# scale-lab/MTLoRA

Hardware: AMD Instinct MI355X
Metric: images/sec (train step) Swin-T/448 r=64 4-task (higher is better)
Workload: dtype bf16; 1 GPU; BASELINE configs[1]: Swin-T 448, 4 tasks (semseg,normals,sal,human_parts), r_shared=64 r_task=4 scale4; train step (fwd+loss+bwd+clip+AdamW), dropout .05, drop_path .2; per_gpu_batch=32, global_batch=32, img_size=448, parallelism=dp1, trainable_params=8344634, allreduce_bytes=0

## Files before the change

include/mtlora_hip.h:

```cpp
#ifndef MTLORA_HIP_H
#define MTLORA_HIP_H

#include <stdint.h>

#ifdef __cplusplus
extern "C" {
#endif

#define MTLORA_ABI_VERSION 12
#define MTLORA_MAX_TASKS 8

typedef enum mtlora_dtype {
    MTLORA_F32 = 0,
    MTLORA_BF16 = 1,
    MTLORA_F16 = 2,
    MTLORA_U8 = 3
} mtlora_dtype;

typedef enum mtlora_status {
    MTLORA_OK = 0,
    MTLORA_ERR_DTYPE = -1,
    MTLORA_ERR_SHAPE = -2,
    MTLORA_ERR_ALIGN = -3,
    MTLORA_ERR_NULL = -4,
// ... 23 lines not shown
    int32_t T;
    int32_t r_s;
    int32_t r_t[MTLORA_MAX_TASKS];
    float scale_s;
    float scale_t[MTLORA_MAX_TASKS];
    int32_t has_x_tasks;
    float dropout_p;
    uint64_t seed;
    const uint64_t* seed_offset;
    int32_t bwd_phase;
    int32_t sel_stream;
    int32_t sel_dense;
    int32_t sel_tn;
    int32_t sel_projk;
    int32_t max_cu;
    const void* packed;
    int32_t hid;
    int32_t hid_pad_;
    const void* hid_ptr;
} mtlora_linear_desc;

#define MTLORA_HID_FWD_BASE 1
#define MTLORA_HID_P_GIVEN 2
#define MTLORA_HID_Q_GIVEN 4

int64_t mtlora_linear_ctx_bytes(const mtlora_linear_desc* d);

int64_t mtlora_linear_packed_bytes(const mtlora_linear_desc* d);
int mtlora_linear_pack(const mtlora_linear_desc* d, const float* A_s, const float* B_s, const float* const* A_t,
                       const float* const* B_t, void* packed, int64_t packed_bytes, void* stream);
int64_t mtlora_linear_pack_entry_bytes(void);
int mtlora_linear_pack_entry(const mtlora_linear_desc* d, const float* A_s, const float* B_s, const float* const* A_t,
                             const float* const* B_t, void* packed, int64_t packed_bytes, void* entry_host);
int mtlora_linear_pack_table(const void* table_dev, int n_entries, int dtype, void* stream);
int64_t mtlora_linear_bwd_scratch_bytes(const mtlora_linear_desc* d);

int mtlora_linear_fwd(const mtlora_linear_desc* d, const void* x, const void* const* x_t, const void* W,
                      const float* bias, const float* A_s, const float* B_s, const float* const* A_t,
                      const float* const* B_t, void* y_s, void* const* y_t, void* ctx, int64_t ctx_bytes,
                      void* stream);

int mtlora_linear_bwd(const mtlora_linear_desc* d, const void* x, const void* const* x_t, const void* Wt,
                      const void* dy_s, const void* const* dy_t, const void* ctx, int64_t ctx_bytes, void* dx,
                      void* const* dx_t, float* dA_s, float* dB_s, float* const* dA_t, float* const* dB_t,
                      void* scratch, int64_t scratch_bytes, void* stream);

int mtlora_linear_fwd_gelu(const mtlora_linear_desc* d, const void* x, const void* const* x_t, const void* W,
                           const float* bias, const float* A_s, const float* B_s, const float* const* A_t,
                           const float* const* B_t, void* y_s, void* const* y_t, void* a_s, void* const* a_t, void* ctx,
                           int64_t ctx_bytes, void* stream);

int mtlora_linear_bwd_gelu(const mtlora_linear_desc* d, const void* x, const void* const* x_t, const void* Wt,
                           const void* dy_s, const void* const* dy_t, const void* ctx, int64_t ctx_bytes, void* dx,
                           void* const* dx_t, float* dA_s, float* dB_s, float* const* dA_t, float* const* dB_t,
                           void* scratch, int64_t scratch_bytes, const void* h_s, const void* const* h_t, void* stream);

int mtlora_mlp_hid_supported(const mtlora_linear_desc* d1, const mtlora_linear_desc* d2);
int64_t mtlora_mlp_hid_fwd_scratch_bytes(const mtlora_linear_desc* d1, const mtlora_linear_desc* d2);
int64_t mtlora_mlp_hid_bwd_scratch_bytes(const mtlora_linear_desc* d1, const mtlora_linear_desc* d2);
int mtlora_mlp_hid_proj(const mtlora_linear_desc* d1, const mtlora_linear_desc* d2, const void* h_base, const void* ctx1,
                        void* ctx2, void* scratch, int64_t scratch_bytes, void* stream);
int mtlora_mlp_hid_bwd(const mtlora_linear_desc* d1, const mtlora_linear_desc* d2, const void* h_base, const void* dh_s,
                       const void* ctx1, const void* ctx2, const void* scratch2, void* scratch1, void* g, float* const* dB1_t,
                       float* const* dA2_t, void* part, int64_t part_bytes, void* stream);

int64_t mtlora_gemm_tn_scratch_bytes(int64_t M, int Na, int Nb);
int mtlora_gemm_tn(const void* a, const void* b, float* out, int64_t M, int Na, int Nb, int64_t lda, int64_t ldb,
                   int dtype, void* scratch, int64_t scratch_bytes, void* stream);

typedef struct mtlora_attn_desc {
    int64_t B;
    int32_t H, W;
    int32_t window_size;
    int32_t shift;
    int32_t num_heads;
    int32_t head_dim;
    int32_t image_layout;
    int32_t dtype;
    float scale;
    float mask_value;
} mtlora_attn_desc;

int64_t mtlora_window_attn_bwd_scratch_bytes(const mtlora_attn_desc* d);

int mtlora_window_attn_fwd(const mtlora_attn_desc* d, const void* qkv, const float* bias, const float* mask,
                           const int32_t* mask_ids, void* out, void* stream);
int mtlora_window_attn_bwd(const mtlora_attn_desc* d, const void* qkv, const float* bias, const float* mask,
                           const int32_t* mask_ids, const void* dout, void* dqkv, float* dbias, void* scratch,
                           int64_t scratch_bytes, void* stream);

typedef struct mtlora_attn_dropout {
    float p;
    uint64_t seed;
    const uint64_t* seed_offset;
} mtlora_attn_dropout;
int mtlora_window_attn_drop_fwd(const mtlora_attn_desc* d, const mtlora_attn_dropout* drop, const void* qkv, const float* bias,
                                const float* mask, const int32_t* mask_ids, void* out, void* stream);
int mtlora_window_attn_drop_bwd(const mtlora_attn_desc* d, const mtlora_attn_dropout* drop, const void* qkv, const float* bias,
                                const float* mask, const int32_t* mask_ids, const void* dout, void* dqkv, float* dbias, void* scratch,
                                int64_t scratch_bytes, void* stream);

int mtlora_layernorm_fwd(const void* x, const float* gamma, const float* beta, void* y, float* mean, float* rstd,
                         int64_t M, int64_t C, float eps, int x_dtype, int y_dtype, int merge_h, int merge_w, void* stream);
int64_t mtlora_layernorm_bwd_scratch_bytes(int64_t M, int64_t C, int x_dtype);
int mtlora_layernorm_bwd(const void* dy, const void* x, const float* gamma, const float* mean, const float* rstd,
                         void* dx, float* dgamma, float* dbeta, int64_t M, int64_t C, int x_dtype, int dy_dtype,
                         void* scratch, int64_t scratch_bytes, const void* dx_addend, int merge_h, int merge_w, void* stream);

int mtlora_residual_layernorm_fwd(const void* shortcut, const void* branch, const float* scale, int64_t B, const float* gamma,
                                  const float* beta, void* x_new, void* y, float* mean, float* rstd, int64_t M, int64_t C,
                                  float eps, int x_dtype, int y_dtype, void* stream);
int mtlora_residual_layernorm_bwd(const void* dy, const void* x_new, const float* gamma, const float* mean, const float* rstd,
                                  void* d_shortcut, void* d_branch, float* dgamma, float* dbeta, const float* scale,
                                  int64_t B, int64_t M, int64_t C, int x_dtype, int dy_dtype, void* scratch,
                                  int64_t scratch_bytes, const void* dx_addend, void* stream);

int64_t mtlora_layernorm_multi_bwd_scratch_bytes(int n, int64_t M, int64_t C, int x_dtype);
int mtlora_layernorm_multi_fwd(int n, const void* const* x, const float* gamma, const float* beta, void* const* y,
                               float* const* mean, float* const* rstd, int64_t M, int64_t C, float eps, int x_dtype, int y_dtype,
                               int merge_h, int merge_w, void* stream);
int mtlora_layernorm_multi_bwd(int n, const void* const* dy, const void* const* x, const float* gamma, const float* const* mean,
                               const float* const* rstd, void* const* dx, float* dgamma, float* dbeta, int64_t M, int64_t C,
                               int x_dtype, int dy_dtype, void* scratch, int64_t scratch_bytes, const void* const* dx_addend,
                               int merge_h, int merge_w, void* stream);

int mtlora_residual_layernorm_streams_fwd(int n, const void* const* res, const void* const* branch, const float* scale,
                                          int64_t B, const float* gamma, const float* beta, void* const* x_new, void* const* y,
                                          float* const* mean, float* const* rstd, int64_t M, int64_t C, float eps, int x_dtype,
                                          int y_dtype, int merge_h, int merge_w, void* stream);
int mtlora_residual_layernorm_streams_bwd(int n, const void* const* dy, const void* const* x_new, const float* gamma,
                                          const float* const* mean, const float* const* rstd, void* const* d_res,
                                          void* const* d_branch, float* dgamma, float* dbeta, const float* scale, int64_t B,
                                          int64_t M, int64_t C, int x_dtype, int dy_dtype, void* scratch, int64_t scratch_bytes,
                                          const void* const* dx_addend, int merge_h, int merge_w, void* stream);

int mtlora_residual_layernorm_multi_fwd(int n, const void* shortcut, const void* const* branch, const float* scale, int64_t B,
                                        const float* gamma, const float* beta, void* const* x_new, void* const* y,
                                        float* const* mean, float* const* rstd, int64_t M, int64_t C, float eps, int x_dtype,
                                        int y_dtype, void* stream);
int mtlora_residual_layernorm_multi_bwd(int n, const void* const* dy, const void* const* x_new, const float* gamma,
                                        const float* const* mean, const float* const* rstd, const void* const* dx_addend,
                                        void* d_shortcut, void* const* d_branch, float* dgamma, float* dbeta, const float* scale,
                                        int64_t B, int64_t M, int64_t C, int x_dtype, int dy_dtype, void* scratch,
                                        int64_t scratch_bytes, void* stream);

int64_t mtlora_bn_scratch_bytes(int64_t R, int64_t C, int dtype);
int mtlora_bn_relu_fwd(const void* x, const float* gamma, const float* beta, float* running_mean, float* running_var,
                       float momentum, float eps, int relu, void* y, float* save_mean, float* save_rstd,
                       float* save_scale, float* save_shift, int64_t R, int64_t C, int dtype, void* scratch,
                       int64_t scratch_bytes, void* stream);
int mtlora_bn_relu_bwd(const void* dy, const void* x, const float* save_mean, const float* save_rstd,
                       const float* save_scale, const float* save_shift, int relu, void* dx, float* dgamma, float* dbeta,
                       int64_t R, int64_t C, int dtype, void* scratch, int64_t scratch_bytes, void* stream);

int mtlora_residual_droppath_fwd(int n, const void* const* res, const void* const* y, void* const* out,
                                 const float* scale, int64_t M, int64_t C, int64_t B, int res_dtype, int y_dtype,
                                 void* stream);
int mtlora_residual_droppath_bwd(int n, const void* const* g, void* const* dy, void* dres, const float* scale,
                                 int64_t M, int64_t C, int64_t B, int res_dtype, int y_dtype, void* stream);

int64_t mtlora_upsample_loss_partials(int64_t B, int h, int w, int scale);
int mtlora_upsample_loss(int kind, const void* low, const float* label, const float* stat, void* dlow, float* partials,
                         int64_t B, int h, int w, int C, int scale, int dtype, float ignore_index, void* stream);

int mtlora_upsample_metrics_sizes(int kind, int64_t B, int h, int w, int C, int scale, int64_t* n_int64,
                                  int64_t* n_float_partials);
// ... 188 lines not shown
```

mtlora_amd/_lib.py:

```python
from __future__ import annotations

import ctypes
import os
from ctypes import POINTER, Structure, c_char_p, c_double, c_float, c_int, c_int32, c_int64, c_uint64, c_void_p

import torch

MAX_TASKS = 8
ABI_VERSION = 12
F32, BF16, F16, U8 = 0, 1, 2, 3
_DT = {torch.float32: F32, torch.bfloat16: BF16, torch.float16: F16}

_HERE = os.path.dirname(os.path.abspath(__file__))
LIB_PATH = os.path.join(_HERE, "csrc", "libmtlora_hip.so")


class LinearDesc(Structure):
    _fields_ = [("M", c_int64), ("K", c_int64), ("N", c_int64), ("dtype", c_int32), ("mode", c_int32),
                ("T", c_int32), ("r_s", c_int32), ("r_t", c_int32 * MAX_TASKS), ("scale_s", c_float),
                ("scale_t", c_float * MAX_TASKS), ("has_x_tasks", c_int32), ("dropout_p", c_float),
                ("seed", c_uint64), ("seed_offset", c_void_p), ("bwd_phase", c_int32),
                ("sel_stream", c_int32), ("sel_dense", c_int32), ("sel_tn", c_int32), ("sel_projk", c_int32),
                ("max_cu", c_int32), ("packed", c_void_p),
                ("hid", c_int32), ("hid_pad_", c_int32), ("hid_ptr", c_void_p)]
# ... 40 lines not shown
    _fields_ = [("kind", c_int64), ("warmup_t", c_int64), ("warmup_prefix", c_int64), ("t_initial", c_int64), ("decay_t", c_int64),
                ("n_milestones", c_int64), ("milestones", c_int64 * 16), ("warmup_lr_init", c_double), ("lr_min", c_double),
                ("lr_min_rate", c_double), ("decay_rate", c_double), ("gamma", c_double), ("base_lr", c_double * 16)]


class IngestJob(Structure):
    _fields_ = [("src", c_void_p), ("dst", c_void_p), ("kind", c_int32), ("src_dtype", c_int32), ("C", c_int32),
                ("reserved", c_int32)]


class AugmentJob(Structure):
    _fields_ = [("src", c_void_p), ("dst", c_void_p), ("kind", c_int32), ("flags", c_int32)]


class MeterSource(Structure):
    _fields_ = [("src", c_void_p), ("dtype", c_int32), ("reserved", c_int32), ("weight", c_double), ("period", c_int64)]


METER_MAX_SLOTS, METER_F32, METER_F64 = 64, 0, 1
INGEST_MAX_JOBS = 8
AUGMENT_IMAGE_CUBIC_U8, AUGMENT_CLASS_NEAREST_U8, AUGMENT_NORMALS_CUBIC_F32, AUGMENT_DEPTH_NEAREST_F32 = 0, 1, 2, 3
AUGMENT_GEOM_BITS, AUGMENT_FLAG_NO_RENORM = 24, 1
INGEST_IMAGE, INGEST_CLASS, INGEST_CLASS_ALLZERO_IGNORE, INGEST_NORMALS, INGEST_DEPTH = 0, 1, 2, 3, 4

ADAMW_CHUNK, ADAMW_MAX_GROUPS, ADAMW_CTRL_WORDS = 4096, 16, 64
ADAMW_GROUPS_DEV_BYTES = 1152
ADAMW_CTRL_MICRO, ADAMW_CTRL_UPDATED = 5, 6
ADAMW_MAX_ACCUM_STEPS = 1 << 24
LR_MAX_MILESTONES = 16
LR_COSINE, LR_STEP, LR_LINEAR, LR_MULTISTEP = 1, 2, 3, 4
ADAMW_SCHED_COUNT_OFFSET, ADAMW_SCHED_LR_OFFSET, ADAMW_SCHED_DEV_BYTES = 344, 352, 480
SNAPSHOT_CHUNK = 32768

PROF_KINDS = 24


class ProfSummary(Structure):
    _fields_ = [("count", c_int64 * PROF_KINDS), ("ms", ctypes.c_double * PROF_KINDS),
                ("alg_bytes", ctypes.c_double * PROF_KINDS), ("s8d_bytes", ctypes.c_double * PROF_KINDS),
                ("flops", ctypes.c_double * PROF_KINDS)]


PtrArr = c_void_p * MAX_TASKS
PtrArr9 = c_void_p * (MAX_TASKS + 1)

_SIGS = {
    "mtlora_version": (c_int, []),
    "mtlora_error_string": (c_char_p, [c_int]),
    "mtlora_roll_and_window_partition_forward": (c_int, [c_void_p, c_void_p, c_int64, c_int64, c_int64, c_int64, c_int, c_int, c_int, c_void_p]),
    "mtlora_roll_and_window_partition_backward": (c_int, [c_void_p, c_void_p, c_int64, c_int64, c_int64, c_int64, c_int, c_int, c_int, c_void_p]),
    "mtlora_window_merge_and_roll_forward": (c_int, [c_void_p, c_void_p, c_int64, c_int64, c_int64, c_int64, c_int, c_int, c_int, c_void_p]),
    "mtlora_window_merge_and_roll_backward": (c_int, [c_void_p, c_void_p, c_int64, c_int64, c_int64, c_int64, c_int, c_int, c_int, c_void_p]),
    "mtlora_linear_ctx_bytes": (c_int64, [POINTER(LinearDesc)]),
    "mtlora_linear_bwd_scratch_bytes": (c_int64, [POINTER(LinearDesc)]),
    "mtlora_linear_packed_bytes": (c_int64, [POINTER(LinearDesc)]),
    "mtlora_linear_pack": (c_int, [POINTER(LinearDesc), c_void_p, c_void_p, POINTER(c_void_p), POINTER(c_void_p), c_void_p, c_int64,
                                   c_void_p]),
    "mtlora_linear_pack_entry_bytes": (c_int64, []),
    "mtlora_linear_pack_entry": (c_int, [POINTER(LinearDesc), c_void_p, c_void_p, POINTER(c_void_p), POINTER(c_void_p), c_void_p, c_int64,
                                         c_void_p]),
    "mtlora_linear_pack_table": (c_int, [c_void_p, c_int, c_int, c_void_p]),
    "mtlora_linear_fwd": (c_int, [POINTER(LinearDesc), c_void_p, POINTER(c_void_p), c_void_p, c_void_p, c_void_p, c_void_p,
                                  POINTER(c_void_p), POINTER(c_void_p), c_void_p, POINTER(c_void_p), c_void_p, c_int64,
                                  c_void_p]),
    "mtlora_linear_bwd": (c_int, [POINTER(LinearDesc), c_void_p, POINTER(c_void_p), c_void_p, c_void_p, POINTER(c_void_p),
                                  c_void_p, c_int64, c_void_p, POINTER(c_void_p), c_void_p, c_void_p, POINTER(c_void_p),
                                  POINTER(c_void_p), c_void_p, c_int64, c_void_p]),
    "mtlora_gemm_tn_scratch_bytes": (c_int64, [c_int64, c_int, c_int]),
    "mtlora_gemm_tn": (c_int, [c_void_p, c_void_p, c_void_p, c_int64, c_int, c_int, c_int64, c_int64, c_int, c_void_p, c_int64,
                               c_void_p]),
    "mtlora_linear_fwd_gelu": (c_int, [POINTER(LinearDesc), c_void_p, POINTER(c_void_p), c_void_p, c_void_p, c_void_p, c_void_p,
                                       POINTER(c_void_p), POINTER(c_void_p), c_void_p, POINTER(c_void_p), c_void_p,
                                       POINTER(c_void_p), c_void_p, c_int64, c_void_p]),
    "mtlora_linear_bwd_gelu": (c_int, [POINTER(LinearDesc), c_void_p, POINTER(c_void_p), c_void_p, c_void_p, POINTER(c_void_p),
                                       c_void_p, c_int64, c_void_p, POINTER(c_void_p), c_void_p, c_void_p, POINTER(c_void_p),
                                       POINTER(c_void_p), c_void_p, c_int64, c_void_p, POINTER(c_void_p), c_void_p]),
    "mtlora_mlp_hid_supported": (c_int, [POINTER(LinearDesc), POINTER(LinearDesc)]),
    "mtlora_mlp_hid_bwd_scratch_bytes": (c_int64, [POINTER(LinearDesc), POINTER(LinearDesc)]),
    "mtlora_mlp_hid_fwd_scratch_bytes": (c_int64, [POINTER(LinearDesc), POINTER(LinearDesc)]),
    "mtlora_mlp_hid_proj": (c_int, [POINTER(LinearDesc), POINTER(LinearDesc), c_void_p, c_void_p, c_void_p, c_void_p, c_int64, c_void_p]),
    "mtlora_mlp_hid_bwd": (c_int, [POINTER(LinearDesc), POINTER(LinearDesc), c_void_p, c_void_p, c_void_p, c_void_p, c_void_p, c_void_p,
                                   c_void_p, POINTER(c_void_p), POINTER(c_void_p), c_void_p, c_int64, c_void_p]),
    "mtlora_window_attn_bwd_scratch_bytes": (c_int64, [POINTER(AttnDesc)]),
    "mtlora_window_attn_fwd": (c_int, [POINTER(AttnDesc), c_void_p, c_void_p, c_void_p, c_void_p, c_void_p, c_void_p]),
    "mtlora_window_attn_bwd": (c_int, [POINTER(AttnDesc), c_void_p, c_void_p, c_void_p, c_void_p, c_void_p, c_void_p,
                                       c_void_p, c_void_p, c_int64, c_void_p]),
    "mtlora_window_attn_drop_fwd": (c_int, [POINTER(AttnDesc), POINTER(AttnDropout), c_void_p, c_void_p, c_void_p, c_void_p, c_void_p,
                                            c_void_p]),
    "mtlora_window_attn_drop_bwd": (c_int, [POINTER(AttnDesc), POINTER(AttnDropout), c_void_p, c_void_p, c_void_p, c_void_p, c_void_p,
                                            c_void_p, c_void_p, c_void_p, c_int64, c_void_p]),
    "mtlora_layernorm_fwd": (c_int, [c_void_p, c_void_p, c_void_p, c_void_p, c_void_p, c_void_p, c_int64, c_int64, c_float,
                                     c_int, c_int, c_int, c_int, c_void_p]),
    "mtlora_layernorm_bwd_scratch_bytes": (c_int64, [c_int64, c_int64, c_int]),
    "mtlora_residual_layernorm_fwd": (c_int, [c_void_p, c_void_p, c_void_p, c_int64, c_void_p, c_void_p, c_void_p, c_void_p,
                                              c_void_p, c_void_p, c_int64, c_int64, c_float, c_int, c_int, c_void_p]),
    "mtlora_layernorm_multi_bwd_scratch_bytes": (c_int64, [c_int, c_int64, c_int64, c_int]),
    "mtlora_layernorm_multi_fwd": (c_int, [c_int, POINTER(c_void_p), c_void_p, c_void_p, POINTER(c_void_p), POINTER(c_void_p),
                                           POINTER(c_void_p), c_int64, c_int64, c_float, c_int, c_int, c_int, c_int, c_void_p]),
    "mtlora_layernorm_multi_bwd": (c_int, [c_int, POINTER(c_void_p), POINTER(c_void_p), c_void_p, POINTER(c_void_p),
                                           POINTER(c_void_p), POINTER(c_void_p), c_void_p, c_void_p, c_int64, c_int64, c_int,
                                           c_int, c_void_p, c_int64, POINTER(c_void_p), c_int, c_int, c_void_p]),
    "mtlora_residual_layernorm_streams_fwd": (c_int, [c_int, POINTER(c_void_p), POINTER(c_void_p), c_void_p, c_int64, c_void_p,
                                                      c_void_p, POINTER(c_void_p), POINTER(c_void_p), POINTER(c_void_p),
                                                      POINTER(c_void_p), c_int64, c_int64, c_float, c_int, c_int, c_int, c_int,
                                                      c_void_p]),
    "mtlora_residual_layernorm_streams_bwd": (c_int, [c_int, POINTER(c_void_p), POINTER(c_void_p), c_void_p, POINTER(c_void_p),
                                                      POINTER(c_void_p), POINTER(c_void_p), POINTER(c_void_p), c_void_p, c_void_p,
                                                      c_void_p, c_int64, c_int64, c_int64, c_int, c_int, c_void_p, c_int64,
                                                      POINTER(c_void_p), c_int, c_int, c_void_p]),
    "mtlora_residual_layernorm_multi_fwd": (c_int, [c_int, c_void_p, POINTER(c_void_p), c_void_p, c_int64, c_void_p, c_void_p,
                                                    POINTER(c_void_p), POINTER(c_void_p), POINTER(c_void_p), POINTER(c_void_p),
                                                    c_int64, c_int64, c_float, c_int, c_int, c_void_p]),
    "mtlora_residual_layernorm_multi_bwd": (c_int, [c_int, POINTER(c_void_p), POINTER(c_void_p), c_void_p, POINTER(c_void_p),
                                                    POINTER(c_void_p), POINTER(c_void_p), c_void_p, POINTER(c_void_p), c_void_p,
                                                    c_void_p, c_void_p, c_int64, c_int64, c_int64, c_int, c_int, c_void_p, c_int64,
                                                    c_void_p]),
    "mtlora_residual_layernorm_bwd": (c_int, [c_void_p, c_void_p, c_void_p, c_void_p, c_void_p, c_void_p, c_void_p, c_void_p,
                                              c_void_p, c_void_p, c_int64, c_int64, c_int64, c_int, c_int, c_void_p, c_int64,
                                              c_void_p, c_void_p]),
    "mtlora_layernorm_bwd": (c_int, [c_void_p, c_void_p, c_void_p, c_void_p, c_void_p, c_void_p, c_void_p, c_void_p,
                                     c_int64, c_int64, c_int, c_int, c_void_p, c_int64, c_void_p, c_int, c_int, c_void_p]),
    "mtlora_bn_scratch_bytes": (c_int64, [c_int64, c_int64, c_int]),
    "mtlora_bn_relu_fwd": (c_int, [c_void_p, c_void_p, c_void_p, c_void_p, c_void_p, c_float, c_float, c_int, c_void_p,
                                   c_void_p, c_void_p, c_void_p, c_void_p, c_int64, c_int64, c_int, c_void_p, c_int64,
                                   c_void_p]),
    "mtlora_bn_relu_bwd": (c_int, [c_void_p, c_void_p, c_void_p, c_void_p, c_void_p, c_void_p, c_int, c_void_p, c_void_p,
                                   c_void_p, c_int64, c_int64, c_int, c_void_p, c_int64, c_void_p]),
    "mtlora_residual_droppath_fwd": (c_int, [c_int, POINTER(c_void_p), POINTER(c_void_p), POINTER(c_void_p), c_void_p,
                                             c_int64, c_int64, c_int64, c_int, c_int, c_void_p]),
    "mtlora_residual_droppath_bwd": (c_int, [c_int, POINTER(c_void_p), POINTER(c_void_p), c_void_p, c_void_p, c_int64,
                                             c_int64, c_int64, c_int, c_int, c_void_p]),
    "mtlora_upsample_loss_partials": (c_int64, [c_int64, c_int, c_int, c_int]),
    "mtlora_colsum_scratch_bytes": (c_int64, [c_int64, c_int64]),
    "mtlora_colsum": (c_int, [c_void_p, c_int64, c_int64, c_int, c_void_p, c_void_p, c_int64, c_void_p]),
    "mtlora_label_stat_scratch_bytes": (c_int64, [c_int64]),
    "mtlora_label_stat": (c_int, [c_void_p, c_int64, c_int, c_float, c_void_p, c_void_p, c_int64, c_void_p]),
    "mtlora_upsample_loss": (c_int, [c_int, c_void_p, c_void_p, c_void_p, c_void_p, c_void_p, c_int64, c_int, c_int, c_int,
                                     c_int, c_int, ctypes.c_float, c_void_p]),
    "mtlora_upsample_metrics_sizes": (c_int, [c_int, c_int64, c_int, c_int, c_int, c_int, POINTER(c_int64), POINTER(c_int64)]),
    "mtlora_upsample_metrics": (c_int, [c_int, c_void_p, c_void_p, c_void_p, c_void_p, c_void_p, c_int64, c_int, c_int, c_int,
                                        c_int, c_int, ctypes.c_float, c_void_p]),
    "mtlora_upsample_predict": (c_int, [c_int, c_void_p, c_void_p, c_int64, c_int, c_int, c_int, c_int, c_int, c_int, c_void_p]),
    "mtlora_upsample_cl_fwd": (c_int, [c_void_p, c_void_p, c_int64, c_int, c_int, c_int, c_int, c_int64, c_int, c_void_p]),
    "mtlora_upsample_cl_bwd": (c_int, [c_void_p, c_void_p, c_int64, c_int, c_int, c_int, c_int, c_int64, c_int, c_void_p]),
    "mtlora_block_save_bytes": (c_int64, [POINTER(BlockDesc)]),
    "mtlora_block_fwd_tmp_bytes": (c_int64, [POINTER(BlockDesc)]),
    "mtlora_block_bwd_scratch_bytes": (c_int64, [POINTER(BlockDesc)]),
    "mtlora_block_fwd": (c_int, [POINTER(BlockDesc), POINTER(BlockParams), c_void_p, c_void_p, c_void_p, c_void_p, c_void_p, c_int64,
                                 c_void_p, c_int64, c_void_p]),
    "mtlora_block_bwd": (c_int, [POINTER(BlockDesc), POINTER(BlockParams), c_void_p, c_void_p, c_void_p, c_void_p, c_void_p, c_void_p,
                                 c_int64, POINTER(BlockGrads), c_void_p, c_int64, c_int, c_void_p]),
    "mtlora_adamw_sizes": (c_int, [c_int64, POINTER(c_int64), POINTER(c_int64), POINTER(c_int64), POINTER(c_int64)]),
    "mtlora_adamw_table": (c_int, [c_int64, POINTER(c_int64), POINTER(c_int32), POINTER(c_void_p), POINTER(c_void_p), POINTER(c_void_p),
                                   c_void_p, c_int64]),
    "mtlora_adamw_update": (c_int, [c_void_p, c_void_p, c_int64, c_int64, POINTER(AdamwGroup), c_int, c_float, c_void_p, c_void_p,
                                    c_void_p, c_void_p, c_float, c_float, c_int, c_void_p, c_int64, c_void_p]),
    "mtlora_adamw_update_dev": (c_int, [c_void_p, c_void_p, c_int64, c_int64, c_void_p, c_int, c_float, c_void_p, c_void_p,
                                        c_void_p, c_void_p, c_double, c_double, c_int, c_void_p, c_int64, c_void_p]),
    "mtlora_adamw_accum_layout": (c_int, [c_int64, POINTER(c_int64), POINTER(c_int64), POINTER(c_int64)]),
    "mtlora_adamw_accum_update_dev": (c_int, [c_void_p, c_void_p, c_int64, c_int64, c_void_p, c_int, c_float, c_void_p, c_void_p,
                                              c_void_p, c_void_p, c_double, c_double, c_int, c_void_p, c_int64, c_void_p, c_void_p,
                                              c_int, c_void_p]),
    "mtlora_lr_schedule_check": (c_int, [POINTER(LrSchedule), c_int]),
    "mtlora_lr_schedule_value": (c_int, [POINTER(LrSchedule), c_int, c_int, c_int64, POINTER(c_double)]),
    "mtlora_adamw_sched_update_dev": (c_int, [c_void_p, c_void_p, c_int64, c_int64, c_void_p, c_int, c_float, c_void_p, c_void_p,
                                              c_void_p, c_void_p, c_double, c_double, c_int, c_void_p, c_int64, c_void_p, c_void_p,
# ... 98 lines not shown
```

mtlora_amd/csrc/attention.hip:

```cpp
#include <atomic>
#include <cmath>
#include <type_traits>

#include "dispatch.h"

namespace {

#ifndef MTL_ATTN_FWD_WPS
#define MTL_ATTN_FWD_WPS 2
#endif
#ifndef MTL_ATTN_BWD_WPS
#define MTL_ATTN_BWD_WPS 1
#endif
constexpr int AN = 64;
constexpr int HD = 32;

template <typename T>
struct AC;
template <>
struct AC<bf16> {
    static constexpr int KT_D = 1;
    static constexpr int KT_N = 2;
    static constexpr int RS = 80;
    static constexpr int VPR = 4;
// ... 688 lines not shown
                    __builtin_amdgcn_sched_barrier(0);
                    attn_keep_tile(dc, rh, sj * 32 + h4, [&](int r, bool keep) __attribute__((always_inline)) {
                        dp[sj][r] = keep ? dp[sj][r] * p.keep_scale : 0.f;
                        kept |= keep ? 1u << (16 * sj + r) : 0u;
                    });
                }
                __builtin_amdgcn_sched_barrier(0);
            }
            float D = 0.f;
#pragma unroll
            for (int sj = 0; sj < 2; ++sj)
#pragma unroll
                for (int r = 0; r < 16; ++r) D += pt[sj][r] * dp[sj][r];
            D += __shfl_xor(D, 32);
#pragma unroll
            for (int sj = 0; sj < 2; ++sj)
#pragma unroll
                for (int r = 0; r < 16; ++r) {
                    const float ds = pt[sj][r] * (dp[sj][r] - D);
                    dp[sj][r] = ds;
                    dbacc[si][sj][r] += ds;
                }
            if constexpr (DROP) {
#pragma unroll
                for (int sj = 0; sj < 2; ++sj)
#pragma unroll
                    for (int r = 0; r < 16; ++r) pt[sj][r] = ((kept >> (16 * sj + r)) & 1u) ? pt[sj][r] * p.keep_scale : 0.f;
            }
            __builtin_amdgcn_wave_barrier();
            img_store<T>(sPi, pt, lane);
            img_store<T>(sDi, dp, lane);
            f32x16 dq;
            zero(dq);
#pragma unroll
            for (int kt = 0; kt < AC<T>::KT_N; ++kt) {
                Frag<T> fk = colfrag(sK, kt, lane, p.N, (T*)nullptr);
                Frag<T> fs = regfrag(dp, kt, (T*)nullptr);
                mtl_mma(fk, fs, dq);
            }
            store_dt_lds<T>(stg, gb, tok + si * 32, p.N - si * 32, dq, p.scale, lane);
            __builtin_amdgcn_s_waitcnt(0xc07f);
            __builtin_amdgcn_wave_barrier();
#pragma unroll
            for (int kq = 0; kq < KQ; ++kq) {
                Frag<T> fq = colfrag(sQ, si * KQ + kq, lane, p.N, (T*)nullptr);
                Frag<T> fo = colfrag(sO, si * KQ + kq, lane, p.N, (T*)nullptr);
#pragma unroll
                for (int sj = 0; sj < 2; ++sj) {
                    Frag<T> fds = imgfrag(sDi, sj * 32, kq, lane, (T*)nullptr);
                    Frag<T> fp = imgfrag(sPi, sj * 32, kq, lane, (T*)nullptr);
                    mtl_mma(fq, fds, dk[sj]);
                    mtl_mma(fo, fp, dv[sj]);
                }
            }
        }
#pragma unroll
        for (int sj = 0; sj < 2; ++sj) {
            if (sj * 32 < p.N) {
                store_dt_lds<T>(stg, gb + p.C, tok + sj * 32, p.N - sj * 32, dk[sj], p.scale, lane);
                store_dt_lds<T>(stg, gb + 2 * p.C, tok + sj * 32, p.N - sj * 32, dv[sj], 1.f, lane);
            }
        }
    }
    float* dst = p.dbias_part + ((int64_t)g * p.nH + head) * p.N * p.N;
#pragma unroll
    for (int si = 0; si < 2; ++si)
#pragma unroll
        for (int sj = 0; sj < 2; ++sj)
#pragma unroll
            for (int r = 0; r < 16; ++r) {
                const int i = si * 32 + (lane & 31), j = sj * 32 + (r & 3) + 8 * (r >> 2) + h4;
                if (i < p.N && j < p.N) dst[j * p.N + i] = dbacc[si][sj][r];
            }
}
template <typename T, bool DENSE>
__global__ __launch_bounds__(64, MTL_ATTN_BWD_WPS) void k_attn_bwd(const AttnParams p) {
    attn_bwd_body<T, DENSE, false>(p);
}
template <typename T, bool DENSE>
__global__ __launch_bounds__(64, MTL_ATTN_BWD_WPS) void k_attn_drop_bwd(const AttnDropParams p) {
    attn_bwd_body<T, DENSE, true>(p);
}

__global__ __launch_bounds__(256) void k_dbias_reduce(const float* part, float* dbias, int G, int nH, int N) {
    __shared__ float sm[4][64];
    const int lane = threadIdx.x & 63, wave = threadIdx.x >> 6;
    const int total = nH * N * N;
    const int idx = blockIdx.x * 64 + lane;
    float a0 = 0.f, a1 = 0.f;
    if (idx < total) {
        int g = wave;
        for (; g + 4 < G; g += 8) {
            a0 += part[(int64_t)g * total + idx];
            a1 += part[(int64_t)(g + 4) * total + idx];
        }
        for (; g < G; g += 4) a0 += part[(int64_t)g * total + idx];
    }
    sm[wave][lane] = a0 + a1;
    __syncthreads();
    if (wave == 0 && idx < total) {
        const int h = idx / (N * N), rem = idx % (N * N);
        const int j = rem / N, i = rem % N;
        dbias[((int64_t)h * N + i) * N + j] = (sm[0][lane] + sm[1][lane]) + (sm[2][lane] + sm[3][lane]);
    }
}

constexpr int WIDE_MAX_N = 144;

int check(const mtlora_attn_desc* d) {
    if (!d) return MTLORA_ERR_NULL;
    if (!mtl_dtype_in(d->dtype, MTL_DT_ALL)) return MTLORA_ERR_DTYPE;
    if (d->head_dim != HD) return MTLORA_ERR_UNSUPPORTED;
    if (d->window_size <= 0 || d->window_size * d->window_size > WIDE_MAX_N) return MTLORA_ERR_UNSUPPORTED;
    if (d->B < 0 || d->H <= 0 || d->W <= 0 || d->num_heads <= 0) return MTLORA_ERR_SHAPE;
    if (d->H % d->window_size || d->W % d->window_size) return MTLORA_ERR_SHAPE;
    if (d->shift < 0 || d->shift >= d->window_size) return MTLORA_ERR_SHAPE;
    if (d->B * d->H * d->W >= ((int64_t)1 << 31)) return MTLORA_ERR_SHAPE;
    if ((int64_t)d->H * d->W * 3 * d->num_heads * d->head_dim * 4 >= ((int64_t)1 << 31)) return MTLORA_ERR_SHAPE;
    return MTLORA_OK;
}

static int groups_for(size_t lds_bytes, int cap, int nH, int64_t n_windows) {
    int per_cu = (int)((160 * 1024) / (lds_bytes + 512));
    if (per_cu > cap) per_cu = cap;
    if (per_cu < 1) per_cu = 1;
    int64_t G = ((int64_t)256 * per_cu) / nH;
    if (G > n_windows) G = n_windows;
    if (G < 1) G = 1;
    return (int)G;
}

struct AttnSizes {
    size_t rs, img, stg;
};
static AttnSizes attn_sizes(int dtype) {
    return mtl_dispatch_f32_bf16(dtype, [](auto t) -> AttnSizes {
        return {AC<typename decltype(t)::type>::RS, IMG<typename decltype(t)::type>::RS, STG<typename decltype(t)::type>::BYTES};
    });
}
static size_t narrow_lds_bytes(int dtype, int N, bool bwd) {
    const AttnSizes z = attn_sizes(dtype);
    const size_t ib = (img_rows_h(N) * z.rs + 15) / 16 * 16;
    return (bwd ? 4 * ib + 2 * 32 * z.img : 3 * ib) + 2 * AN * 4 + z.stg + (dtype == MTLORA_F32 ? (size_t)N * bias_stride_c(N) * 4 : 0);
}

int bwd_groups(const mtlora_attn_desc* d) {
    const int64_t nwin = d->B * (d->H / d->window_size) * (d->W / d->window_size);
    return groups_for(narrow_lds_bytes(d->dtype, d->window_size * d->window_size, true), 4 * MTL_ATTN_BWD_WPS, d->num_heads, nwin);
}

AttnParams make_params(const mtlora_attn_desc* d) {
    AttnParams p = {};
    p.H = d->H;
    p.W = d->W;
    p.ws = d->window_size;
    p.shift = d->shift;
    p.nH = d->num_heads;
    p.N = d->window_size * d->window_size;
    p.C = d->num_heads * d->head_dim;
    p.nWx = d->W / d->window_size;
    p.nWy = d->H / d->window_size;
    p.n_windows = d->B * p.nWx * p.nWy;
    p.image_layout = d->image_layout;
    p.scale = d->scale;
    return p;
}

#include "attention_wide.h"

template <typename T, bool DENSE>
static const void* narrow_kernel(const AttnParams&, bool bwd) {
    return bwd ? reinterpret_cast<const void*>(k_attn_bwd<T, DENSE>) : reinterpret_cast<const void*>(k_attn_fwd<T, DENSE>);
}
template <typename T, bool DENSE>
static const void* narrow_kernel(const AttnDropParams&, bool bwd) {
    return bwd ? reinterpret_cast<const void*>(k_attn_drop_bwd<T, DENSE>) : reinterpret_cast<const void*>(k_attn_drop_fwd<T, DENSE>);
}
template <typename P>
static void narrow_launch(int dtype, bool bwd, const P& p, size_t lds, hipStream_t s) {
    const bool dense = p.mask && !p.mask_ids;
    const void* k = mtl_dispatch_dtype(dtype, [&](auto t) {
        return dense ? narrow_kernel<typename decltype(t)::type, true>(p, bwd) : narrow_kernel<typename decltype(t)::type, false>(p, bwd);
    });
    void* args[] = {const_cast<P*>(&p)};
    (void)hipLaunchKernel(k, dim3((unsigned)(p.G * p.nH)), dim3(64), args, lds, s);
}

template <typename P>
static int attn_fwd_run(const mtlora_attn_desc* d, P& p, hipStream_t s) {
    const double ab = 4.0 * mtl_elem_size(d->dtype) * (double)p.n_windows * p.N * p.C;
    MtlProfScope prof(PK_ATTN_FWD, ab, s, ab, 4.0 * (double)p.n_windows * p.N * p.N * p.C);
    if (p.N > AN) {
        const int wst = wide_fwd(d, p, s);
        if (wst != MTLORA_OK) return wst;
        MTL_CHECK_LAUNCH();
        return MTLORA_OK;
    }
    const size_t lds = narrow_lds_bytes(d->dtype, p.N, false);
    p.G = groups_for(lds, 4 * MTL_ATTN_FWD_WPS, p.nH, p.n_windows);
    narrow_launch(d->dtype, false, p, lds, s);
    MTL_CHECK_LAUNCH();
    return MTLORA_OK;
}
template <typename P>
static int attn_bwd_run(const mtlora_attn_desc* d, P& p, float* dbias, hipStream_t s) {
    {
        const double ab = 7.0 * mtl_elem_size(d->dtype) * (double)p.n_windows * p.N * p.C;
        MtlProfScope prof(PK_ATTN_BWD, ab, s, ab, 8.0 * (double)p.n_windows * p.N * p.N * p.C);
        if (p.N > AN) {
            const int wst = wide_bwd(d, p, s);
            if (wst != MTLORA_OK) return wst;
        } else {
            p.G = bwd_groups(d);
            narrow_launch(d->dtype, true, p, narrow_lds_bytes(d->dtype, p.N, true), s);
        }
    }
    const int total = p.nH * p.N * p.N;
    hipLaunchKernelGGL(k_dbias_reduce, dim3((unsigned)((total + 63) / 64)), dim3(256), 0, s, (const float*)p.dbias_part, dbias, p.G,
                       p.nH, p.N);
    MTL_CHECK_LAUNCH();
    return MTLORA_OK;
}

static int drop_setup(const mtlora_attn_desc* d, const mtlora_attn_dropout* dr, bool plain, AttnDropParams& p, bool& on) {
    on = false;
    if (plain) return MTLORA_OK;
    if (!dr) return MTLORA_ERR_NULL;
    if (!std::isfinite(dr->p) || dr->p < 0.f || dr->p >= 1.f) return MTLORA_ERR_SHAPE;
    p.drop = mtl_make_dropout(dr->p, dr->seed, dr->seed_offset);
    on = p.drop.enabled();
    p.keep_scale = on ? 1.f / (1.f - dr->p) : 1.f;
    const int64_t nwin = d->B * (d->H / d->window_size) * (d->W / d->window_size);
    if (on && nwin * d->num_heads * d->window_size * d->window_size >= ((int64_t)1 << 32)) return MTLORA_ERR_SHAPE;
    return MTLORA_OK;
}

static int attn_fwd_entry(const mtlora_attn_desc* d, const mtlora_attn_dropout* dr, bool plain, const void* qkv, const float* bias,
                          const float* mask, const int32_t* mask_ids, void* out, void* stream) {
    int st = check(d);
    if (st != MTLORA_OK) return st;
    AttnDropParams p = {};
    bool drop_on;
    if ((st = drop_setup(d, dr, plain, p, drop_on)) != MTLORA_OK) return st;
    if (mtl_any_null({qkv, bias, out})) return MTLORA_ERR_NULL;
    if (mtl_any_misaligned({qkv, out})) return MTLORA_ERR_ALIGN;
    static_cast<AttnParams&>(p) = make_params(d);
    if (p.n_windows == 0) return MTLORA_OK;
    p.qkv = qkv;
    p.bias = bias;
    p.mask = mask;
    p.mask_ids = mask_ids;
    p.mask_value = d->mask_value;
    p.out = out;
    return drop_on ? attn_fwd_run(d, p, (hipStream_t)stream) : attn_fwd_run(d, static_cast<AttnParams&>(p), (hipStream_t)stream);
}

static int attn_bwd_entry(const mtlora_attn_desc* d, const mtlora_attn_dropout* dr, bool plain, const void* qkv, const float* bias,
                          const float* mask, const int32_t* mask_ids, const void* dout, void* dqkv, float* dbias, void* scratch,
                          int64_t scratch_bytes, void* stream) {
    int st = check(d);
    if (st != MTLORA_OK) return st;
    AttnDropParams p = {};
    bool drop_on;
    if ((st = drop_setup(d, dr, plain, p, drop_on)) != MTLORA_OK) return st;
    if (mtl_any_null({qkv, bias, dout, dqkv, dbias, scratch})) return MTLORA_ERR_NULL;
    if (mtl_any_misaligned({qkv, dout, dqkv, scratch})) return MTLORA_ERR_ALIGN;
    if (scratch_bytes < mtlora_window_attn_bwd_scratch_bytes(d) - 256) return MTLORA_ERR_WORKSPACE;
    static_cast<AttnParams&>(p) = make_params(d);
    hipStream_t s = (hipStream_t)stream;
    if (p.n_windows == 0) {
        mtl_zero_async(dbias, (size_t)p.nH * p.N * p.N * 4, s);
        return MTLORA_OK;
    }
    p.qkv = qkv;
    p.bias = bias;
    p.mask = mask;
    p.mask_ids = mask_ids;
    p.mask_value = d->mask_value;
    p.dout = dout;
    p.dqkv = dqkv;
    p.dbias_part = reinterpret_cast<float*>(scratch);
    return drop_on ? attn_bwd_run(d, p, dbias, s) : attn_bwd_run(d, static_cast<AttnParams&>(p), dbias, s);
}

}

extern "C" {

int64_t mtlora_window_attn_bwd_scratch_bytes(const mtlora_attn_desc* d) {
    if (check(d) != MTLORA_OK) return -1;
    const int N = d->window_size * d->window_size;
    if (N > AN) return (int64_t)wide_groups(d) * d->num_heads * N * N * 4 + 256;
    return (int64_t)bwd_groups(d) * d->num_heads * N * N * 4 + 256;
}

int mtlora_window_attn_fwd(const mtlora_attn_desc* d, const void* qkv, const float* bias, const float* mask,
                           const int32_t* mask_ids, void* out, void* stream) {
    return attn_fwd_entry(d, nullptr, true, qkv, bias, mask, mask_ids, out, stream);
}

int mtlora_window_attn_bwd(const mtlora_attn_desc* d, const void* qkv, const float* bias, const float* mask,
                           const int32_t* mask_ids, const void* dout, void* dqkv, float* dbias, void* scratch,
                           int64_t scratch_bytes, void* stream) {
    return attn_bwd_entry(d, nullptr, true, qkv, bias, mask, mask_ids, dout, dqkv, dbias, scratch, scratch_bytes, stream);
}

int mtlora_window_attn_drop_fwd(const mtlora_attn_desc* d, const mtlora_attn_dropout* drop, const void* qkv, const float* bias,
                                const float* mask, const int32_t* mask_ids, void* out, void* stream) {
    return attn_fwd_entry(d, drop, false, qkv, bias, mask, mask_ids, out, stream);
}

int mtlora_window_attn_drop_bwd(const mtlora_attn_desc* d, const mtlora_attn_dropout* drop, const void* qkv, const float* bias,
                                const float* mask, const int32_t* mask_ids, const void* dout, void* dqkv, float* dbias, void* scratch,
                                int64_t scratch_bytes, void* stream) {
    return attn_bwd_entry(d, drop, false, qkv, bias, mask, mask_ids, dout, dqkv, dbias, scratch, scratch_bytes, stream);
}
}
```

Measured before the change: 1163 images/sec.

## Add two-wave split-row window attention backward kernel for large workloads

Adds a new window-attention backward kernel that splits each window's 64 query rows across two waves per 128-thread block. The waves share Q/K/V/dO tiles in LDS, exchange partial dK/dV through LDS, and fold the bias into the MMA accumulator through an identity-matrix multiply. The goal is more parallelism and better latency hiding for bf16/f16 windows with 32<N<=64 when windows×heads is large. A runtime selector picks the new form above a threshold, with an override exposed through a new API. Scratch sizing now covers the larger of the two forms' group counts.

After: 1101 images/sec. 5.3% lower.

```diff
diff --git a/include/mtlora_hip.h b/include/mtlora_hip.h
--- a/include/mtlora_hip.h
+++ b/include/mtlora_hip.h
@@ -129,6 +129,7 @@
 } mtlora_attn_desc;
 
 int64_t mtlora_window_attn_bwd_scratch_bytes(const mtlora_attn_desc* d);
+int mtlora_window_attn_bwd_set_form(int form);
 
 int mtlora_window_attn_fwd(const mtlora_attn_desc* d, const void* qkv, const float* bias, const float* mask,
                            const int32_t* mask_ids, void* out, void* stream);
diff --git a/mtlora_amd/_lib.py b/mtlora_amd/_lib.py
--- a/mtlora_amd/_lib.py
+++ b/mtlora_amd/_lib.py
@@ -146,6 +146,7 @@
     "mtlora_mlp_hid_bwd": (c_int, [POINTER(LinearDesc), POINTER(LinearDesc), c_void_p, c_void_p, c_void_p, c_void_p, c_void_p, c_void_p,
                                    c_void_p, POINTER(c_void_p), POINTER(c_void_p), c_void_p, c_int64, c_void_p]),
     "mtlora_window_attn_bwd_scratch_bytes": (c_int64, [POINTER(AttnDesc)]),
+    "mtlora_window_attn_bwd_set_form": (c_int, [c_int]),
     "mtlora_window_attn_fwd": (c_int, [POINTER(AttnDesc), c_void_p, c_void_p, c_void_p, c_void_p, c_void_p, c_void_p]),
     "mtlora_window_attn_bwd": (c_int, [POINTER(AttnDesc), c_void_p, c_void_p, c_void_p, c_void_p, c_void_p, c_void_p,
                                        c_void_p, c_void_p, c_int64, c_void_p]),
diff --git a/mtlora_amd/csrc/attention.hip b/mtlora_amd/csrc/attention.hip
--- a/mtlora_amd/csrc/attention.hip
+++ b/mtlora_amd/csrc/attention.hip
@@ -794,6 +794,288 @@
     attn_bwd_body<T, DENSE, true>(p);
 }
 
+template <typename T>
+struct BiasHalf {
+    Frag<f16> bf[2];
+    float c, maskv;
+};
+template <typename T>
+__device__ __forceinline__ void bias_init_half(BiasHalf<T>& B, const AttnParams& p, int head, int si, int lane) {
+    const float* src = p.bias + (int64_t)head * p.N * p.N;
+    const float inv = 1.f / p.scale;
+    const int rl = lane & 31, h = lane >> 5;
+    const int i = si * 32 + rl;
+#pragma unroll
+    for (int sj = 0; sj < 2; ++sj)
+#pragma unroll
+        for (int t = 0; t < 2; ++t) {
+            float f[8];
+#pragma unroll
+            for (int e = 0; e < 8; ++e) {
+                const int j = sj * 32 + 16 * t + 8 * h + e;
+                f[e] = j < p.N ? (i < p.N ? src[i * p.N + j] * inv : 0.f) : pad_big<T>();
+            }
+            B.bf[sj].v[t] = u32x4{mtl_pk2<f16>(f[0], f[1]), mtl_pk2<f16>(f[2], f[3]), mtl_pk2<f16>(f[4], f[5]), mtl_pk2<f16>(f[6], f[7])};
+        }
+    B.c = p.scale * 1.4426950408889634f;
+    B.maskv = p.mask_value * inv;
+}
+template <typename T, bool DENSE>
+__device__ __forceinline__ void scores_half(f32x16 (&st)[2], const unsigned char* sK, const unsigned char* sQ, int si, const AttnParams& p,
+                                            const BiasHalf<T>& B, const int* srid, bool masked, int wm, int lane) {
+    zero(st[0]);
+    zero(st[1]);
+    {
+        Frag<f16> idf;
+        const int rl = lane & 31, h = lane >> 5;
+        const uint32_t one = 0x3C00u;
+#pragma unroll
+        for (int t = 0; t < 2; ++t) {
+            uint32_t w[4];
+#pragma unroll
+            for (int e2 = 0; e2 < 4; ++e2) {
+                const int k0 = 16 * t + 8 * h + 2 * e2;
+                w[e2] = (k0 == rl ? one : 0u) | (k0 + 1 == rl ? one << 16 : 0u);
+            }
+            idf.v[t] = u32x4{w[0], w[1], w[2], w[3]};
+        }
+#pragma unroll
+        for (int sj = 0; sj < 2; ++sj) mtl_mma(idf, B.bf[sj], st[sj]);
+    }
+    Frag<T> fq = rowfrag<T>(sQ, si, 0, lane, p.N);
+#pragma unroll
+    for (int sj = 0; sj < 2; ++sj) {
+        Frag<T> fk = rowfrag<T>(sK, sj, 0, lane, p.N);
+        mtl_mma(fk, fq, st[sj]);
+    }
+    if (DENSE || masked) {
+        const int i = si * 32 + (lane & 31);
+        const bool iv = i < p.N;
+        const int ic = iv ? i : p.N - 1;
+        const int h4 = 4 * (lane >> 5);
+        const int rid_i = srid[ic];
+        const float* mrow = DENSE ? p.mask + ((int64_t)wm * p.N + ic) * p.N : nullptr;
+        const float inv = DENSE ? 1.f / p.scale : 0.f;
+#pragma unroll
+        for (int sj = 0; sj < 2; ++sj) {
+            __builtin_amdgcn_sched_barrier(0);
+#pragma unroll
+            for (int r = 0; r < 16; ++r) {
+                const int j = sj * 32 + (r & 3) + 8 * (r >> 2) + h4;
+                const int jc = j < p.N ? j : p.N - 1;
+                float add;
+                if constexpr (DENSE)
+                    add = mrow[jc] * inv;
+                else
+                    add = srid[jc] != rid_i ? B.maskv : 0.f;
+                st[sj][r] += (iv && j < p.N) ? add : 0.f;
+            }
+        }
+        __builtin_amdgcn_sched_barrier(0);
+    }
+}
+constexpr int BWD2_XB = 2 * 4 * 64 * 16;
+__device__ __forceinline__ void xchg_store(unsigned char* x, const f32x16 (&a)[2], int lane) {
+#pragma unroll
+    for (int sj = 0; sj < 2; ++sj)
+#pragma unroll
+        for (int q = 0; q < 4; ++q)
+            *reinterpret_cast<f32x4*>(x + ((sj * 4 + q) * 64 + lane) * 16) = f32x4{a[sj][4 * q], a[sj][4 * q + 1], a[sj][4 * q + 2], a[sj][4 * q + 3]};
+}
+__device__ __forceinline__ void xchg_add(f32x16 (&a)[2], const unsigned char* x, int lane) {
+#pragma unroll
+    for (int sj = 0; sj < 2; ++sj)
+#pragma unroll
+        for (int q = 0; q < 4; ++q) {
+            const f32x4 v = *reinterpret_cast<const f32x4*>(x + ((sj * 4 + q) * 64 + lane) * 16);
+#pragma unroll
+            for (int e = 0; e < 4; ++e) a[sj][4 * q + e] += v[e];
+        }
+}
+
+template <typename T, bool DENSE, bool DROP, typename P>
+__device__ __forceinline__ void attn_bwd2_body(const P p) {
+    static_assert(sizeof(T) == 2, "16-bit types only");
+    constexpr int RS = AC<T>::RS, HB = 32 * IMG<T>::RS;
+    static_assert(2 * HB >= BWD2_XB, "a wave's two hand-over images hold its outgoing partial");
+    extern __shared__ __attribute__((aligned(16))) unsigned char smem[];
+    const int IB = ((img_rows(p.N) * RS + 15) / 16) * 16;
+    const int si = __builtin_amdgcn_readfirstlane((int)(threadIdx.x >> 6));
+    unsigned char* sQ = smem;
+    unsigned char* sK = smem + IB;
+    unsigned char* sV = smem + 2 * IB;
+    unsigned char* sO = smem + 3 * IB;
+    unsigned char* sPi = smem + 4 * IB + si * 2 * HB;
+    unsigned char* sDi = sPi + HB;
+    unsigned char* sPeer = smem + 4 * IB + (1 - si) * 2 * HB;
+    int* tok = reinterpret_cast<int*>(smem + 4 * IB + 4 * HB);
+    int* srid = tok + AN;
+    const int lane0 = threadIdx.x & 63, lane = lane0;
+    const int64_t L = xcd_remap(blockIdx.x, gridDim.x);
+    const int head = (int)(L % p.nH);
+    const int g = (int)(L / p.nH);
+    const int nWimg = p.nWx * p.nWy;
+    const T* qkv = reinterpret_cast<const T*>(p.qkv) + head * HD;
+    const T* dout = reinterpret_cast<const T*>(p.dout) + head * HD;
+    T* dqkv = reinterpret_cast<T*>(p.dqkv) + head * HD;
+    const int C3 = 3 * p.C;
+    BiasHalf<T> B;
+    bias_init_half<T>(B, p, head, si, lane);
+    f32x16 dbacc[2];
+    zero(dbacc[0]);
+    zero(dbacc[1]);
+    const int h4 = 4 * (lane >> 5);
+    const RowIds<T> ids = row_ids<T>(p, lane);
+    const int lane_tyx = pack_tyx(p, lane < p.N ? lane : 0);
+    [[maybe_unused]] DropoutCfg dc;
+    if constexpr (DROP) dc = attn_drop_cfg(p);
+    for (int64_t w = g; w < p.n_windows; w += p.G) {
+        int lane = attn_opaque_lane<true>(lane0);
+        const int wm = (int)(w % nWimg);
+        const WinPos wq = win_pos(p, w);
+        T* gb = dqkv + wq.base * C3;
+        {
+            RowRegs<T> ra, rb;
+            int offa[AC<T>::VPR], offb[AC<T>::VPR];
+            row_offsets<T>(offa, p, wq, ids, C3, lane);
+            row_offsets<T>(offb, p, wq, ids, si ? p.C : C3, lane);
+            const T* wb = qkv + wq.base * C3;
+            load_rows<T>(ra, si ? wb + 2 * p.C : wb, offa);
+            load_rows<T>(rb, si ? dout + wq.base * p.C : wb + p.C, offb);
+            int rid = 0;
+            if (si == 0) rid = (p.mask_ids && lane < p.N) ? p.mask_ids[wm * p.N + lane] : 0;
+            __syncthreads();
+            if (si == 0) {
+                tok[lane] = lane < p.N ? token_at(p, wq, lane, lane_tyx) * C3 : 0;
+                srid[lane] = rid;
+            }
+            store_rows<T>(si ? sV : sQ, ra, p.N, lane);
+            store_rows<T>(si ? sO : sK, rb, p.N, lane);
+            __syncthreads();
+        }
+        __builtin_amdgcn_sched_barrier(0);
+        lane = attn_opaque_lane<true>(lane0);
+        const int rid_l = srid[lane];
+        const bool masked = __ballot(lane < p.N && rid_l != __builtin_amdgcn_readfirstlane(rid_l)) != 0ull;
+
+        f32x16 dk[2], dv[2];
+        {
+            f32x16 pt[2];
+            scores_half<T, DENSE>(pt, sK, sQ, si, p, B, srid, masked, wm, lane);
+            (void)softmax_t<true, false>(pt, B.c);
+            f32x16 dp[2];
+            zero(dp[0]);
+            zero(dp[1]);
+            {
+                Frag<T> fo = rowfrag<T>(sO, si, 0, lane, p.N);
+#pragma unroll
+                for (int sj = 0; sj < 2; ++sj) {
+                    Frag<T> fv = rowfrag<T>(sV, sj, 0, lane, p.N);
+                    mtl_mma(fv, fo, dp[sj]);
+                }
+            }
+            [[maybe_unused]] uint32_t kept = 0u;
+            if constexpr (DROP) {
+                const uint32_t rh = attn_drop_rowhash(dc, p, w, head, si * 32 + (lane & 31));
+#pragma unroll
+                for (int sj = 0; sj < 2; ++sj) {
+                    __builtin_amdgcn_sched_barrier(0);
+                    attn_keep_tile(dc, rh, sj * 32 + h4, [&](int r, bool keep) __attribute__((always_inline)) {
+                        dp[sj][r] = keep ? dp[sj][r] * p.keep_scale : 0.f;
+                        kept |= keep ? 1u << (16 * sj + r) : 0u;
+                    });
+                }
+                __builtin_amdgcn_sched_barrier(0);
+            }
+            float D = 0.f;
+#pragma unroll
+            for (int sj = 0; sj < 2; ++sj)
+#pragma unroll
+                for (int r = 0; r < 16; ++r) D += pt[sj][r] * dp[sj][r];
+            D += __shfl_xor(D, 32);
+#pragma unroll
+            for (int sj = 0; sj < 2; ++sj)
+#pragma unroll
+                for (int r = 0; r < 16; ++r) {
+                    const float ds = pt[sj][r] * (dp[sj][r] - D);
+                    dp[sj][r] = ds;
+                    dbacc[sj][r] += ds;
+                }
+            if constexpr (DROP) {
+#pragma unroll
+                for (int sj = 0; sj < 2; ++sj)
+#pragma unroll
+                    for (int r = 0; r < 16; ++r) pt[sj][r] = ((kept >> (16 * sj + r)) & 1u) ? pt[sj][r] * p.keep_scale : 0.f;
+            }
+            img_store<T>(sPi, pt, lane);
+            img_store<T>(sDi, dp, lane);
+            f32x16 dq;
+            zero(dq);
+#pragma unroll
+            for (int kt = 0; kt < 2; ++kt) {
+                Frag<T> fk = colfrag(sK, kt, lane, p.N, (T*)nullptr);
+                Frag<T> fs = regfrag(dp, kt, (T*)nullptr);
+                mtl_mma(fk, fs, dq);
+            }
+            __builtin_amdgcn_s_waitcnt(0xc07f);
+            __builtin_amdgcn_wave_barrier();
+            __builtin_amdgcn_sched_barrier(0);
+            lane = attn_opaque_lane<true>(lane0);
+            zero(dk[0]);
+            zero(dk[1]);
+            zero(dv[0]);
+            zero(dv[1]);
+            {
+                Frag<T> fq = colfrag(sQ, si, lane, p.N, (T*)nullptr);
+                Frag<T> fo = colfrag(sO, si, lane, p.N, (T*)nullptr);
+#pragma unroll
+                for (int sj = 0; sj < 2; ++sj) {
+                    Frag<T> fds = imgfrag(sDi, sj * 32, 0, lane, (T*)nullptr);
+                    Frag<T> fp = imgfrag(sPi, sj * 32, 0, lane, (T*)nullptr);
+                    mtl_mma(fq, fds, dk[sj]);
+                    mtl_mma(fo, fp, dv[sj]);
+                }
+            }
+            __builtin_amdgcn_wave_barrier();
+            store_dt_lds<T>(sPi, gb, tok + si * 32, p.N - si * 32, dq, p.scale, lane);
+        }
+        if (si == 0)
+            xchg_store(sPi, dv, lane);
+        else
+            xchg_store(sPi, dk, lane);
+        __syncthreads();
+        lane = attn_opaque_lane<true>(lane0);
+        unsigned char* stg = smem + si * STG<T>::BYTES;
+        if (si == 0) {
+            xchg_add(dk, sPeer, lane);
+#pragma unroll
+            for (int sj = 0; sj < 2; ++sj)
+                if (sj * 32 < p.N) store_dt_lds<T>(stg, gb + p.C, tok + sj * 32, p.N - sj * 32, dk[sj], p.scale, lane);
+        } else {
+            xchg_add(dv, sPeer, lane);
+#pragma unroll
+            for (int sj = 0; sj < 2; ++sj)
+                if (sj * 32 < p.N) store_dt_lds<T>(stg, gb + 2 * p.C, tok + sj * 32, p.N - sj * 32, dv[sj], 1.f, lane);
+        }
+    }
+    float* dst = p.dbias_part + ((int64_t)g * p.nH + head) * p.N * p.N;
+#pragma unroll
+    for (int sj = 0; sj < 2; ++sj)
+#pragma unroll
+        for (int r = 0; r < 16; ++r) {
+            const int i = si * 32 + (lane & 31), j = sj * 32 + (r & 3) + 8 * (r >> 2) + h4;
+            if (i < p.N && j < p.N) dst[j * p.N + i] = dbacc[sj][r];
+        }
+}
+template <typename T, bool DENSE>
+__global__ __launch_bounds__(128, 2) void k_attn_bwd2(const AttnParams p) {
+    attn_bwd2_body<T, DENSE, false>(p);
+}
+template <typename T, bool DENSE>
+__global__ __launch_bounds__(128, 2) void k_attn_bwd2_drop(const AttnDropParams p) {
+    attn_bwd2_body<T, DENSE, true>(p);
+}
+
 __global__ __launch_bounds__(256) void k_dbias_reduce(const float* part, float* dbias, int G, int nH, int N) {
     __shared__ float sm[4][64];
     const int lane = threadIdx.x & 63, wave = threadIdx.x >> 6;
@@ -856,9 +1138,38 @@
     return (bwd ? 4 * ib + 2 * 32 * z.img : 3 * ib) + 2 * AN * 4 + z.stg + (dtype == MTLORA_F32 ? (size_t)N * bias_stride_c(N) * 4 : 0);
 }
 
-int bwd_groups(const mtlora_attn_desc* d) {
+static size_t bwd2_lds_bytes(int dtype, int N) {
+    const AttnSizes z = attn_sizes(dtype);
+    const size_t ib = (img_rows_h(N) * z.rs + 15) / 16 * 16;
+    return 4 * ib + 4 * 32 * z.img + 2 * AN * 4;
+}
+
+std::atomic<int> g_bwd_form{0};
+#ifndef MTL_ATTN_BWD2_MIN_ITEMS
+#define MTL_ATTN_BWD2_MIN_ITEMS 3072
+#endif
+constexpr int64_t BWD2_MIN_ITEMS = MTL_ATTN_BWD2_MIN_ITEMS;
+static int bwd_form(const mtlora_attn_desc* d) {
+    const int N = d->window_size * d->window_size;
+    if (d->dtype == MTLORA_F32 || N <= 32 || N > AN) return 1;
+    const int f = g_bwd_form.load(std::memory_order_relaxed);
+    if (f) return f;
     const int64_t nwin = d->B * (d->H / d->window_size) * (d->W / d->window_size);
-    return groups_for(narrow_lds_bytes(d->dtype, d->window_size * d->window_size, true), 4 * MTL_ATTN_BWD_WPS, d->num_heads, nwin);
+    return nwin * d->num_heads >= BWD2_MIN_ITEMS ? 2 : 1;
+}
+
+int bwd_groups(const mtlora_attn_desc* d, int form) {
+    const int64_t nwin = d->B * (d->H / d->window_size) * (d->W / d->window_size);
+    const int N = d->window_size * d->window_size;
+    if (form == 2) return groups_for(bwd2_lds_bytes(d->dtype, N), 4, d->num_heads, nwin);
+    return groups_for(narrow_lds_bytes(d->dtype, N, true), 4 * MTL_ATTN_BWD_WPS, d->num_heads, nwin);
+}
+int bwd_groups_max(const mtlora_attn_desc* d) {
+    const int g1 = bwd_groups(d, 1);
+    const int N = d->window_size * d->window_size;
+    if (d->dtype == MTLORA_F32 || N <= 32 || N > AN) return g1;
+    const int g2 = bwd_groups(d, 2);
+    return g1 > g2 ? g1 : g2;
 }
 
 AttnParams make_params(const mtlora_attn_desc* d) {
@@ -888,6 +1199,23 @@
 static const void* narrow_kernel(const AttnDropParams&, bool bwd) {
     return bwd ? reinterpret_cast<const void*>(k_attn_drop_bwd<T, DENSE>) : reinterpret_cast<const void*>(k_attn_drop_fwd<T, DENSE>);
 }
+template <typename T, bool DENSE>
+static const void* bwd2_kernel(const AttnParams&) {
+    return reinterpret_cast<const void*>(k_attn_bwd2<T, DENSE>);
+}
+template <typename T, bool DENSE>
+static const void* bwd2_kernel(const AttnDropParams&) {
+    return reinterpret_cast<const void*>(k_attn_bwd2_drop<T, DENSE>);
+}
+template <typename P>
+static void bwd2_launch(int dtype, const P& p, size_t lds, hipStream_t s) {
+    const bool dense = p.mask && !p.mask_ids;
+    const void* k = mtl_dispatch_dtype16(dtype, [&](auto t) {
+        return dense ? bwd2_kernel<typename decltype(t)::type, true>(p) : bwd2_kernel<typename decltype(t)::type, false>(p);
+    });
+    void* args[] = {const_cast<P*>(&p)};
+    (void)hipLaunchKernel(k, dim3((unsigned)(p.G * p.nH)), dim3(128), args, lds, s);
+}
 template <typename P>
 static void narrow_launch(int dtype, bool bwd, const P& p, size_t lds, hipStream_t s) {
     const bool dense = p.mask && !p.mask_ids;
@@ -922,8 +1250,11 @@
         if (p.N > AN) {
             const int wst = wide_bwd(d, p, s);
             if (wst != MTLORA_OK) return wst;
+        } else if (bwd_form(d) == 2) {
+            p.G = bwd_groups(d, 2);
+            bwd2_launch(d->dtype, p, bwd2_lds_bytes(d->dtype, p.N), s);
         } else {
-            p.G = bwd_groups(d);
+            p.G = bwd_groups(d, 1);
             narrow_launch(d->dtype, true, p, narrow_lds_bytes(d->dtype, p.N, true), s);
         }
     }
@@ -1003,7 +1334,11 @@
     if (check(d) != MTLORA_OK) return -1;
     const int N = d->window_size * d->window_size;
     if (N > AN) return (int64_t)wide_groups(d) * d->num_heads * N * N * 4 + 256;
-    return (int64_t)bwd_groups(d) * d->num_heads * N * N * 4 + 256;
+    return (int64_t)bwd_groups_max(d) * d->num_heads * N * N * 4 + 256;
+}
+
+int mtlora_window_attn_bwd_set_form(int form) {
+    return g_bwd_form.exchange(form == 1 || form == 2 ? form : 0, std::memory_order_relaxed);
 }
 
 int mtlora_window_attn_fwd(const mtlora_attn_desc* d, const void* qkv, const float* bias, const float* mask,
```
